# ICLDisco/parsec

Hardware: NVIDIA H100
Metric: tasks/s (higher is better)
Workload: dtype i32

## Files before the change

### parsec_b200/mca/b200/device_b200.h

```cpp
#ifndef PARSEC_DEVICE_B200_H
#define PARSEC_DEVICE_B200_H

#include "parsec/mca/device/device_gpu.h"

BEGIN_C_DECLS

extern parsec_device_base_component_t parsec_device_b200_component;


int parsec_b200_task_body(parsec_device_gpu_module_t *gpu_device, parsec_gpu_task_t *gpu_task,
                          parsec_gpu_exec_stream_t *gpu_stream,
                          int body, int nb_args, const int *flow_index, const int32_t *iparam, float fparam);

uint64_t parsec_b200_task_result(const parsec_gpu_task_t *gpu_task);

int parsec_b200_is_b200_device(const parsec_device_module_t *device);

typedef struct parsec_b200_stats_s {
    uint64_t tasks_engine;
    uint64_t tasks_lane;
    uint64_t kernel_launches;
    uint64_t released_on_device;
    uint64_t bytes_h2d_kernel, bytes_d2d_kernel, bytes_d2h_kernel;
    uint64_t bytes_h2d_dma, bytes_d2h_dma;
    uint64_t evictions, w2r_copies;
    uint64_t registration_hits;
    uint64_t first_entry_ns, first_task_ns, last_done_ns;
    uint64_t peer_pulls;
    uint64_t peer_detours;
    uint64_t check_mismatches;
    uint64_t manager_entries;
    uint64_t lane_batched;
    uint64_t forwarded;
    uint64_t max_concurrent_callers;
} parsec_b200_stats_t;
int parsec_b200_get_stats(const parsec_device_module_t *device, parsec_b200_stats_t *stats);

END_C_DECLS
#endif
```

### parsec_b200/mca/b200/device_b200_component.c

```c
#include "parsec/parsec_config.h"
#include "parsec/parsec_internal.h"
#include "parsec/utils/mca_param.h"
#include "parsec/utils/debug.h"
#include "parsec/constants.h"
#include "parsec/mca/device/device.h"
#include "parsec/mca/device/device_gpu.h"
#include "parsec/mca/device/b200/device_b200.h"
#include "parsec/mca/device/b200/device_b200_internal.h"

#include <stdlib.h>

int parsec_device_b200_enabled = 0;
int parsec_device_b200_enabled_index = -1;
int parsec_b200_dry_run = 0;
int parsec_b200_memory_block_size = 512 * 1024;
int parsec_b200_memory_percentage = 95;
int parsec_b200_memory_number_of_blocks = -1;
int parsec_b200_cmd_slots = 65536;
int parsec_b200_idle_us = 2000;
int parsec_b200_max_workers = 0;
char *parsec_b200_trace = NULL;
int parsec_b200_nvtx = 0;
int parsec_b200_parallel_completion = 1;
int parsec_b200_stage_window = 32 * 1024 * 1024;
int parsec_b200_registration_cache = 1;
static int b200_mask = -1;

#if !defined(PARSEC_HAVE_MPI)
int parsec_mpi_allow_gpu_memory_communications = 0;
#endif

static int device_b200_component_open(void);
static int device_b200_component_close(void);
static int device_b200_component_query(mca_base_module_2_0_0_t **module, int *priority);
static int device_b200_component_register(void);

parsec_device_base_component_t parsec_device_b200_component = {
    {
        PARSEC_DEVICE_BASE_VERSION_2_0_0,
        "b200",
        "+persistent_kernel+device_release+tma",
        PARSEC_VERSION_MAJOR,
        PARSEC_VERSION_MINOR,
        device_b200_component_open,
        device_b200_component_close,
        device_b200_component_query,
        device_b200_component_register,
        "",
// ... 19 lines not shown
    (void)parsec_mca_param_reg_int_name("device_b200", "mask", "Bit mask of the CUDA devices the component may use",
                                        false, false, -1, &b200_mask);
    (void)parsec_mca_param_reg_int_name("device_b200", "dry_run",
                                        "Host-logic test mode: build modules without touching CUDA; tasks retire in dependency order "
                                        "without running their bodies (the value is the number of pretend devices)",
                                        false, false, 0, &parsec_b200_dry_run);
    (void)parsec_mca_param_reg_int_name("device_b200", "memory_block_size", "Unit of the device heap in bytes",
                                        false, false, 512 * 1024, &parsec_b200_memory_block_size);
    (void)parsec_mca_param_reg_int_name("device_b200", "memory_use", "Percentage of the free GPU memory given to the device heap",
                                        false, false, 95, &parsec_b200_memory_percentage);
    (void)parsec_mca_param_reg_int_name("device_b200", "memory_number_of_blocks",
                                        "Exact number of heap blocks instead of a percentage (-1: use device_b200_memory_use)",
                                        false, false, -1, &parsec_b200_memory_number_of_blocks);
    (void)parsec_mca_param_reg_int_name("device_b200", "cmd_slots", "Capacity of the host->device command ring (tasks in flight)",
                                        false, false, 65536, &parsec_b200_cmd_slots);
    (void)parsec_mca_param_reg_int_name("device_b200", "idle_us", "The persistent kernel parks after this many idle microseconds",
                                        false, false, 2000, &parsec_b200_idle_us);
    (void)parsec_mca_param_reg_int_name("device_b200", "parallel_completion",
                                        "Let the worker pool run __parsec_complete_execution of finished GPU tasks instead of the manager thread",
                                        false, false, 1, &parsec_b200_parallel_completion);
    (void)parsec_mca_param_reg_int_name("device_b200", "stage_window",
                                        "Bytes of stage-in (host or peer to device) allowed in flight before further cold tasks wait",
                                        false, false, 32 * 1024 * 1024, &parsec_b200_stage_window);
    (void)parsec_mca_param_reg_int_name("device_b200", "registration_cache",
                                        "Keep host ranges pinned after memory_unregister and revive them at the next registration of the same range",
                                        false, false, 1, &parsec_b200_registration_cache);
    (void)parsec_mca_param_reg_int_name("device_b200", "max_workers", "Debug: limit the worker CTAs of the persistent kernel (0: all)",
                                        false, false, 0, &parsec_b200_max_workers);
    (void)parsec_mca_param_reg_string_name("device_b200", "trace",
                                           "Write one Chrome-trace JSON file <value>.<device index>.json per device at finalize: every task with the "
                                           "device-clock time a worker CTA started and finished it and the SM it ran on (empty: off)",
                                           false, false, "", &parsec_b200_trace);
    (void)parsec_mca_param_reg_int_name("device_b200", "nvtx",
                                        "Wrap the host side of the device in NVTX ranges (domain \"parsec_b200\": start pass, retire pass, "
                                        "epilog batch) and mark every manager election; what profiling_nvtx.c does for the profiling keys "
                                        "of the reference's stream engine",
                                        false, false, 0, &parsec_b200_nvtx);
    return (0 == parsec_device_b200_enabled && 0 == parsec_b200_dry_run) ? MCA_ERROR : MCA_SUCCESS;
}

static int device_b200_component_open(void)
{
    int ndev = 0;
    if( 0 == parsec_device_b200_enabled && 0 == parsec_b200_dry_run ) return MCA_ERROR;
    if( parsec_b200_dry_run > 0 ) {
        ndev = parsec_b200_dry_run;
// ... 52 lines not shown
```

### parsec_b200/mca/b200/device_b200_internal.h

```cpp
#ifndef PARSEC_DEVICE_B200_INTERNAL_H
#define PARSEC_DEVICE_B200_INTERNAL_H

#include "parsec/mca/device/device_gpu.h"
#include "parsec/mca/device/cuda/device_cuda.h"
#include "parsec/mca/device/b200/device_b200.h"

BEGIN_C_DECLS

extern int parsec_device_b200_enabled, parsec_device_b200_enabled_index, parsec_b200_dry_run;
extern int parsec_b200_memory_block_size, parsec_b200_memory_percentage, parsec_b200_memory_number_of_blocks;
extern int parsec_b200_parallel_completion, parsec_b200_stage_window, parsec_b200_registration_cache;
extern char *parsec_b200_trace;
extern int parsec_b200_nvtx;
extern int parsec_b200_cmd_slots, parsec_b200_idle_us, parsec_b200_max_workers;

int  parsec_b200_device_count(void);
int  parsec_b200_module_init(int dev_id, parsec_device_module_t **module);
int  parsec_b200_module_fini(parsec_device_module_t *device);

END_C_DECLS
#endif
```

### parsec_b200/mca/b200/device_b200_module.c

```c
#include "parsec/parsec_config.h"
#include "parsec/parsec_internal.h"
#include "parsec/sys/atomic.h"
#include "parsec/utils/mca_param.h"
#include "parsec/utils/debug.h"
#include "parsec/utils/zone_malloc.h"
#include "parsec/constants.h"
#include "parsec/data_internal.h"
#include "parsec/scheduling.h"
#include "parsec/execution_stream.h"
#include "parsec/mca/device/device.h"
#include "parsec/mca/device/device_gpu.h"
#include "parsec/mca/device/b200/device_b200.h"
#include "parsec/mca/device/b200/device_b200_internal.h"

#include "pb2_engine.h"
#include "pb2_stream.h"

#include <cuda_runtime_api.h>
#include <stddef.h>
#include <stdlib.h>
#include <string.h>
#include <stdio.h>
#include <limits.h>
#include <time.h>
// ... 24 lines not shown

typedef struct b200_lock_s {
    volatile uint32_t next;    char pad0[60];
    volatile uint32_t serving; char pad1[60];
} b200_lock_t;
static inline void b200_lock(b200_lock_t *l)
{
    const uint32_t t = __atomic_fetch_add(&l->next, 1, __ATOMIC_RELAXED);
    while( __atomic_load_n(&l->serving, __ATOMIC_ACQUIRE) != t ) _mm_pause();
}
static inline void b200_unlock(b200_lock_t *l)
{
    __atomic_store_n(&l->serving, l->serving + 1, __ATOMIC_RELEASE);
}

enum {
    BT_NEW = 0,
    BT_STAGED,
    BT_DMA_IN,
    BT_INFLIGHT,
    BT_LANE,
    BT_DMA_OUT
};

typedef struct b200_task_s {
    parsec_list_item_t   item;
    parsec_gpu_task_t   *gpu_task;
    int32_t              state;
    int32_t              ticket;
    int32_t              body;
    int32_t              prepared;
    int32_t              cmd_built;
    int32_t              recorded;
    int32_t              has_complete_stage;
    uint32_t             dma_out_mask;
    uint64_t             result;
    uint64_t             cold_bytes;
    struct parsec_device_b200_module_s *dev;
    int32_t              is_kernel;
    int32_t              defer_tiles;
    int32_t              ntdesc;
    pb2_task_t           cmd __attribute__((aligned(64)));
    parsec_task_t        proxy __attribute__((aligned(64)));
    int32_t              nb_args;
    int32_t              arg_flow[PB2_MAX_FLOWS];
    int32_t              iparam[3];
    float                fparam;
    uint32_t             peer_src_mask;
    parsec_data_copy_t  *peer_src[MAX_PARAM_COUNT];
    int32_t              custom_stage;
    cudaEvent_t          ev;
    int32_t              ev_dev;
    struct b200_task_s  *next_free;
    struct b200_task_s  *next_done;
    struct { int32_t tile; pb2_tile_t desc; } tdesc[MAX_PARAM_COUNT];
} b200_task_t;

typedef struct b200_host_range_s { char *base; size_t len; char *alias; int lazy; } b200_host_range_t;

typedef struct b200_trace_ev_s {
    char     name[24];
    int32_t  locals[2];
    int32_t  body, smid;
    uint64_t t_start_ns, t_end_ns, cold_bytes;
} b200_trace_ev_t;
#define B200_LINE __attribute__((aligned(64)))
typedef struct parsec_device_b200_module_s {
    parsec_device_cuda_module_t super;
    pb2_engine_t        *engine;
    pb2_stream_t        *stream;
    int                  dry_run;
    char                *slab_base;
    uint8_t             *tile_described;
    b200_task_t * volatile *inbox_ring;
    cudaStream_t         dma_stream;
    parsec_cuda_exec_stream_t *lane;
    uint64_t             first_entry_ns, first_task_ns, last_done_ns;
    volatile int64_t     inbox_tail B200_LINE;
    volatile int32_t     owed B200_LINE;
    volatile int32_t     callers_inside B200_LINE;
    volatile int32_t     max_callers_inside;
    volatile int64_t     epilogs_done B200_LINE;
    b200_lock_t          lru_lock B200_LINE;
    b200_lock_t          alloc_lock B200_LINE;
    volatile int32_t     handed_back B200_LINE;
    volatile int32_t     starter_active B200_LINE;
    volatile int32_t     fatal;
    volatile int32_t     memory_pressure;
    struct b200_task_s * volatile lane_done;
    volatile int32_t     retry_stalled B200_LINE;
    volatile int64_t     cold_inflight B200_LINE;
    volatile int64_t     inbox_head B200_LINE;
    parsec_list_t        stalled B200_LINE;
    parsec_list_t        settled;
    parsec_list_t        cold_q;
    int32_t              nb_cold;
    parsec_list_t        waiting_event;
    int32_t              nb_settled;
    int32_t              nb_stalled;
    int32_t              again_window;
    int32_t              lane_pending;
    uint64_t             n_engine, n_lane, n_settled_by_caller;
    uint64_t             tsc_start[4];
    uint64_t             tsc_s[3];
    parsec_list_t        waiting_out B200_LINE;
    parsec_task_t       *completion_ring;
    b200_task_t         *batch_head;
    int32_t              batch_len;
    int32_t              completed_now;
    int32_t              blocked_spins;
    int32_t              complete_inline;
    int64_t              epilogs_started;
    uint64_t             tsc[8];
    struct b200_trace_ev_s *trace_ev;
    size_t               trace_n, trace_cap;
    pb2_retire_t         retbuf[256];
    parsec_b200_stats_t  st B200_LINE;
} parsec_device_b200_module_t;

static b200_host_range_t *b200_ranges = NULL;
// ... 58 lines not shown
{
    b200_task_t *bt = b200_tl_free;
    if( NULL != bt ) { b200_tl_free = bt->next_free; b200_tl_nfree--; }
    else {
        if( 0 != posix_memalign((void**)&bt, 64, sizeof(b200_task_t)) ) abort();
        memset(bt, 0, sizeof(b200_task_t));
        PARSEC_OBJ_CONSTRUCT(&bt->item, parsec_list_item_t);
        PARSEC_OBJ_CONSTRUCT(&bt->proxy, parsec_task_t);
        bt->proxy.task_class = &b200_completion_tc;
        bt->proxy.priority = INT32_MAX;
        bt->proxy.status = PARSEC_TASK_STATUS_HOOK;
        bt->proxy.chore_mask = 1;
        bt->proxy.selected_chore = 0;
        bt->proxy.selected_device = parsec_mca_device_get(0);
        bt->proxy.load = 0;
        bt->proxy.repo_entry = NULL;
        bt->ev_dev = -1;
    }
    PARSEC_LIST_ITEM_SINGLETON(&bt->item);
    bt->dev = dev;
    bt->gpu_task = gpu_task; bt->state = BT_NEW; bt->ticket = -1; bt->body = -1; bt->nb_args = 0;
    bt->peer_src_mask = 0; bt->dma_out_mask = 0; bt->result = 0; bt->custom_stage = 0; bt->cold_bytes = 0;
    bt->recorded = 0; bt->has_complete_stage = 0; bt->prepared = 0; bt->cmd_built = 0; bt->defer_tiles = 0; bt->ntdesc = 0;
    bt->is_kernel = (NULL == gpu_task) || (PARSEC_GPU_TASK_TYPE_KERNEL == gpu_task->task_type);
    if( NULL != gpu_task ) gpu_task->last_data_check_epoch = (uint64_t)(uintptr_t)bt;
    return bt;
}

static void b200_bt_free(b200_task_t *bt)
{
    bt->gpu_task = NULL;
    if( b200_tl_nfree < B200_TL_CACHE ) { bt->next_free = b200_tl_free; b200_tl_free = bt; b200_tl_nfree++; return; }
    if( bt->ev_dev >= 0 ) (void)cudaEventDestroy(bt->ev);
    free(bt);
}

static inline void b200_cuda_here(parsec_device_b200_module_t *dev)
{
    if( !dev->dry_run ) B200_CUDA(cudaSetDevice(dev->super.cuda_index), "cudaSetDevice", {});
}

static cudaEvent_t b200_bt_event(parsec_device_b200_module_t *dev, b200_task_t *bt)
{
    if( bt->ev_dev != (int32_t)dev->super.cuda_index ) {
        if( bt->ev_dev >= 0 ) (void)cudaEventDestroy(bt->ev);
        bt->ev_dev = -1;
// ... 341 lines not shown
        int transfer_from = parsec_data_start_transfer_ownership_to_copy(original, my, type);
        if( -1 != transfer_from && out->version == src->version && PARSEC_DATA_STATUS_COMPLETE_TRANSFER == out->data_transfer_status ) transfer_from = -1;
        if( NULL == src->device_private ) transfer_from = -1;
        if( (NULL == this_task->data[i].source_repo_entry) && (NULL == original->dc) && (0 == in->version) ) transfer_from = -1;
        if( PARSEC_DATA_STATUS_UNDER_TRANSFER == out->data_transfer_status ) transfer_from = -1;
        mod->required_data_in += original->span;

        pb2_tile_t tile;
        memset(&tile, 0, sizeof tile);
        tile.dev_ptr = out->device_private;
        tile.bytes = (uint32_t)span;
        tile.state = PB2_TILE_VALID;
        tile.src_kind = parsec_mca_device_is_gpu(src->device_index) ? PB2_SRC_PEER : PB2_SRC_HOST;
        char *home = NULL;
        if( NULL != original->device_copies[0] && NULL != original->device_copies[0]->device_private )
            home = b200_device_visible(original->device_copies[0]->device_private, span);
        tile.src_ptr = home;

        if( -1 == transfer_from ) {
            if( src_acquired ) { (void)parsec_atomic_fetch_dec_int32(&src->readers); src_acquired = 0; }
            if( PARSEC_DATA_STATUS_UNDER_TRANSFER != out->data_transfer_status ) {
                out->data_transfer_status = PARSEC_DATA_STATUS_COMPLETE_TRANSFER;
                parsec_data_end_transfer_ownership_to_copy(original, my, type);
            }
            if( PARSEC_FLOW_ACCESS_WRITE & type ) out->version = src->version + 1;
        } else {
            char *visible = (PB2_SRC_PEER == tile.src_kind) ? (char*)src->device_private
                                                            : b200_device_visible(src->device_private, span);
            mod->data_in_from_device[src->device_index] += span;
            mod->nb_data_faults += span;
            bt->cold_bytes += span;
            if( PB2_SRC_PEER == tile.src_kind ) { if( src_detour ) dev->st.peer_detours++; else dev->st.peer_pulls++; }
            if( NULL != visible && !src_detour && !for_lane && !dev->dry_run ) {
                tile.state = PB2_TILE_INVALID;
                tile.src_ptr = visible;
                out->data_transfer_status = PARSEC_DATA_STATUS_UNDER_TRANSFER;
                if( PB2_SRC_PEER == tile.src_kind ) dev->st.bytes_d2d_kernel += span; else dev->st.bytes_h2d_kernel += span;
            } else if( 2 == mode ) {
                out->data_transfer_status = PARSEC_DATA_STATUS_UNDER_TRANSFER;
                used_dma = 1;
            } else if( !dev->dry_run ) {
                b200_cuda_here(dev);
                B200_CUDA(cudaMemcpyAsync(out->device_private, src->device_private, span,
                                          PB2_SRC_PEER == tile.src_kind ? cudaMemcpyDeviceToDevice : cudaMemcpyHostToDevice,
                                          for_lane ? dev->lane->cuda_stream : dev->dma_stream),
                          "stage-in cudaMemcpyAsync", { parsec_atomic_unlock(&original->lock); return PARSEC_HOOK_RETURN_ERROR; });
                out->data_transfer_status = PARSEC_DATA_STATUS_UNDER_TRANSFER;
                dev->st.bytes_h2d_dma += span;
                used_dma = 1;
            } else {
                out->data_transfer_status = PARSEC_DATA_STATUS_UNDER_TRANSFER;
            }
            out->version = (PARSEC_FLOW_ACCESS_WRITE & type) ? src->version + 1 : src->version;
            gpu_task->flow_info[i].source = src;
            if( src_acquired ) { bt->peer_src_mask |= (1u << i); bt->peer_src[i] = src; }
            if( PB2_SRC_PEER == tile.src_kind && PB2_TILE_INVALID == tile.state && NULL != home && (gpu_task->pushout & (1 << i)) ) {
            }
        }
        tile.version = (PARSEC_FLOW_ACCESS_WRITE & type) ? out->version - 1 : out->version;
        if( !for_lane ) {
            const int32_t tid = b200_tile_of(dev, out);
            if( -1 != transfer_from || !dev->tile_described[tid] ) {
                if( 0 != b200_emit_tile(dev, bt, tid, &tile) ) { parsec_atomic_unlock(&original->lock); return PARSEC_HOOK_RETURN_ERROR; }
                dev->tile_described[tid] = 1;
            }
        }
        parsec_atomic_unlock(&original->lock);
    }
    return used_dma;
}

int parsec_b200_task_body(parsec_device_gpu_module_t *gpu_device, parsec_gpu_task_t *gpu_task,
                          parsec_gpu_exec_stream_t *gpu_stream,
                          int body, int nb_args, const int *flow_index, const int32_t *iparam, float fparam)
{
    if( NULL == gpu_device || NULL == gpu_task || nb_args < 0 || nb_args > PB2_MAX_FLOWS || body < 0 || body >= PB2_BODY_MAX )
        return PARSEC_HOOK_RETURN_ERROR;
    for( int a = 0; a < nb_args; a++ )
        if( flow_index[a] < 0 || (uint32_t)flow_index[a] >= gpu_task->nb_flows ) return PARSEC_HOOK_RETURN_ERROR;
    if( parsec_b200_is_b200_device(&gpu_device->super) ) {
        b200_task_t *bt = b200_tl_recording;
        if( NULL == bt || bt->gpu_task != gpu_task ) return PARSEC_HOOK_RETURN_ERROR;
        bt->body = body; bt->nb_args = nb_args;
        for( int a = 0; a < nb_args; a++ ) bt->arg_flow[a] = flow_index[a];
        bt->iparam[0] = iparam ? iparam[0] : 0; bt->iparam[1] = iparam ? iparam[1] : 0; bt->iparam[2] = iparam ? iparam[2] : 0;
        bt->fparam = fparam;
        return PARSEC_HOOK_RETURN_DONE;
    }
    {
        void *ptrs[PB2_MAX_FLOWS] = {NULL, NULL, NULL, NULL};
        uint64_t bytes[PB2_MAX_FLOWS] = {0, 0, 0, 0};
// ... 183 lines not shown
            NULL != gpu_task->ec->data[f].data_out ) bt->dma_out_mask |= (1u << f);
    }
    t->iparam[0] = bt->iparam[0]; t->iparam[1] = bt->iparam[1]; t->iparam[2] = bt->iparam[2]; t->fparam = bt->fparam;
    t->locals[0] = gpu_task->ec->locals[0].value; t->locals[1] = gpu_task->ec->locals[1].value;
    bt->cmd_built = 1;
}

static int b200_push_engine(parsec_device_b200_module_t *dev, b200_task_t *bt)
{
    if( !bt->cmd_built ) b200_build_cmd(dev, bt);
    const int32_t state_before = bt->state;
    bt->state = BT_INFLIGHT;
    int rc = pb2_stream_submit(dev->stream, &bt->cmd, (uint64_t)(uintptr_t)bt, &bt->ticket);
    if( PB2_SUCCESS != rc ) {
        bt->state = state_before;
        if( PB2_ERR_OUT_OF_RESOURCE == rc ) return PARSEC_HOOK_RETURN_AGAIN;
        parsec_warning("device_b200: submit failed: %s", pb2_stream_last_error(dev->stream));
        return PARSEC_HOOK_RETURN_ERROR;
    }
    dev->n_engine++;
    return PARSEC_HOOK_RETURN_DONE;
}

static int b200_prepare_resident(parsec_device_b200_module_t *dev, b200_task_t *bt)
{
    parsec_gpu_task_t *gpu_task = bt->gpu_task;
    parsec_task_t *this_task = gpu_task->ec;
    const uint8_t my = dev->super.super.super.device_index;
    if( NULL == dev->tile_described ) return 0;
    for( uint32_t i = 0; i < gpu_task->nb_flows; i++ ) {
        const parsec_flow_t *flow = gpu_task->flow_info[i].flow;
        if( PARSEC_FLOW_ACCESS_NONE == (PARSEC_FLOW_ACCESS_MASK & flow->flow_flags) ) continue;
        const parsec_data_copy_t *in = this_task->data[i].data_in;
        if( NULL == in ) continue;
        if( in->device_index != my || NULL == in->device_private || NULL == in->original ) return 0;
        if( !dev->tile_described[b200_tile_of(dev, in)] ) return 0;
    }
    for( uint32_t i = 0; i < gpu_task->nb_flows; i++ ) {
        const parsec_flow_t *flow = gpu_task->flow_info[i].flow;
        const uint8_t type = (uint8_t)(flow->flow_flags & PARSEC_FLOW_ACCESS_MASK);
        if( PARSEC_FLOW_ACCESS_NONE == type ) { gpu_task->flow_info[i].flow_span = 0; continue; }
        parsec_data_copy_t *in = this_task->data[i].data_in;
        if( NULL == in ) continue;
        this_task->data[i].data_out = in;
        gpu_task->flow_info[i].source = NULL;
        if( PARSEC_FLOW_ACCESS_WRITE & type ) {
// ... 96 lines not shown

static int b200_start_task(parsec_device_b200_module_t *dev, parsec_execution_stream_t *es, b200_task_t *bt)
{
    parsec_gpu_task_t *gpu_task = bt->gpu_task;
    int rc;
    (void)es;
    dev->again_window = 0;
    if( bt->prepared ) { bt->state = BT_STAGED; return b200_push_engine(dev, bt); }
    if( dev->cold_inflight >= (int64_t)parsec_b200_stage_window && b200_needs_memory(dev, gpu_task) ) { dev->again_window = 1; return PARSEC_HOOK_RETURN_AGAIN; }
    uint64_t c0 = B200_TSC(), c1;
    if( PARSEC_HOOK_RETURN_DONE != (rc = b200_reserve(dev, bt)) ) return rc;
    c1 = B200_TSC(); dev->tsc_start[0] += c1 - c0; c0 = c1;

    const int custom_stage = (NULL != gpu_task->stage_in && gpu_task->stage_in != parsec_default_gpu_stage_in) ||
                             (NULL != gpu_task->stage_out && gpu_task->stage_out != parsec_default_gpu_stage_out);
    const parsec_task_class_t *tc = gpu_task->ec->task_class;
    bt->custom_stage = custom_stage;
    int known_engine = bt->recorded || dev->dry_run || (!custom_stage && parsec_b200_submit_is_engine(gpu_task->submit));

    if( known_engine ) {
        rc = b200_stage_in(dev, bt, 0);
        if( rc < 0 ) return rc;
        c1 = B200_TSC(); dev->tsc_start[1] += c1 - c0; c0 = c1;
        if( bt->cold_bytes ) (void)parsec_atomic_fetch_add_int64(&dev->cold_inflight, (int64_t)bt->cold_bytes);
        int src = 0;
        if( !bt->recorded ) {
            b200_tl_recording = bt;
            src = gpu_task->submit(&dev->super.super, gpu_task, &dev->lane->super);
            b200_tl_recording = NULL;
            bt->recorded = 1;
            bt->has_complete_stage = (NULL != gpu_task->complete_stage);
        }
        if( dev->dry_run && bt->body < 0 ) { bt->body = PB2_BODY_NOP; bt->nb_args = 0; }
        if( src < 0 || bt->body < 0 ) {
            parsec_warning("device_b200: body of task class %s stopped naming an engine body", tc ? tc->name : "?");
            return PARSEC_HOOK_RETURN_ERROR;
        }
        if( rc > 0 ) {
            B200_CUDA(cudaEventRecord(b200_bt_event(dev, bt), dev->dma_stream), "cudaEventRecord", {});
            bt->state = BT_DMA_IN;
            parsec_list_nolock_push_back(&dev->waiting_event, &bt->item);
            return PARSEC_HOOK_RETURN_DONE;
        }
        bt->state = BT_STAGED;
        c1 = B200_TSC(); dev->tsc_start[2] += c1 - c0; c0 = c1;
        rc = b200_push_engine(dev, bt);
        dev->tsc_start[3] += B200_TSC() - c0;
        return rc;
    }

    b200_cuda_here(dev);
    const int user_in = (NULL != gpu_task->stage_in && gpu_task->stage_in != parsec_default_gpu_stage_in);
    rc = b200_stage_in(dev, bt, user_in ? 2 : 1);
    if( rc < 0 ) return rc;
    if( bt->cold_bytes ) (void)parsec_atomic_fetch_add_int64(&dev->cold_inflight, (int64_t)bt->cold_bytes);
    if( user_in ) {
        uint32_t mask = 0;
        for( uint32_t i = 0; i < gpu_task->nb_flows; i++ )
            if( NULL != gpu_task->ec->data[i].data_out && PARSEC_DATA_STATUS_UNDER_TRANSFER == gpu_task->ec->data[i].data_out->data_transfer_status ) mask |= (1u << i);
        if( mask && PARSEC_SUCCESS != gpu_task->stage_in(gpu_task, mask, &dev->lane->super) ) return PARSEC_HOOK_RETURN_ERROR;
// ... 69 lines not shown
        gpu_task->ec = (parsec_task_t*)calloc(1, sizeof(parsec_task_t));
        PARSEC_OBJ_CONSTRUCT(gpu_task->ec, parsec_task_t);
        gpu_task->ec->task_class = &b200_prefetch_tc;
        gpu_task->ec->selected_device = module;
        gpu_task->nb_flows = 1;
        gpu_task->flow_info[0].flow = &b200_prefetch_flow;
        gpu_task->flow_info[0].flow_span = data->span;
        gpu_task->stage_in = parsec_default_gpu_stage_in;
        gpu_task->stage_out = parsec_default_gpu_stage_out;
        gpu_task->submit = b200_prefetch_submit;
        gpu_task->release_device_task = b200_release_pseudo_task;
        PARSEC_DATA_COPY_RETAIN(src);
        gpu_task->ec->data[0].data_in = src;
        (void)b200_kernel_scheduler(module, NULL, gpu_task);
        return PARSEC_SUCCESS;
    }
    default:
        return PARSEC_ERR_NOT_FOUND;
    }
}

static void b200_finish(parsec_device_b200_module_t *dev, parsec_execution_stream_t *es, b200_task_t *bt)
{
    if( bt->cold_bytes ) { (void)parsec_atomic_fetch_add_int64(&dev->cold_inflight, -(int64_t)bt->cold_bytes); bt->cold_bytes = 0; }
    if( !dev->retry_stalled ) dev->retry_stalled = 1;
    if( bt->is_kernel ) { b200_complete(dev, es, bt); return; }
    parsec_gpu_task_t *gpu_task = bt->gpu_task;
    parsec_data_copy_t *out = gpu_task->ec->data[0].data_out;
    if( NULL != out ) {
        parsec_atomic_lock(&out->original->lock);
        if( PARSEC_DATA_STATUS_UNDER_TRANSFER == out->data_transfer_status ) {
            out->data_transfer_status = PARSEC_DATA_STATUS_COMPLETE_TRANSFER;
            parsec_data_end_transfer_ownership_to_copy(out->original, dev->super.super.super.device_index, PARSEC_FLOW_ACCESS_READ);
        }
        if( bt->peer_src_mask & 1u ) (void)parsec_atomic_fetch_dec_int32(&bt->peer_src[0]->readers);
        if( 1 == out->readers ) b200_lru_touch(dev, out);
        (void)parsec_atomic_fetch_dec_int32(&out->readers);
        parsec_atomic_unlock(&out->original->lock);
    }
    b200_bt_free(bt);
    gpu_task->last_data_check_epoch = 0;
    gpu_task->release_device_task(gpu_task);
    dev->completed_now++;
}

static parsec_device_b200_module_t *b200_forward_peer(parsec_device_b200_module_t *dev, const parsec_gpu_task_t *gpu_task)
{
// ... 87 lines not shown
        dev->retry_stalled = 0;
        while( dev->nb_settled > 0 ) {
            if( started >= 512 ) { cut = 1; break; }
            b200_task_t *bt = (b200_task_t*)PARSEC_LIST_ITERATOR_FIRST(&dev->settled);
            parsec_list_item_t *la = PARSEC_LIST_ITERATOR_NEXT(&bt->item);
            if( la != PARSEC_LIST_ITERATOR_END(&dev->settled) ) { la = PARSEC_LIST_ITERATOR_NEXT(la);
                if( la != PARSEC_LIST_ITERATOR_END(&dev->settled) ) { B200_PF(la); B200_PF((const char*)la + offsetof(b200_task_t, cmd)); } }
            parsec_list_nolock_remove(&dev->settled, &bt->item);
            PARSEC_LIST_ITEM_SINGLETON(&bt->item);
            if( BT_NEW == bt->state ) bt->state = BT_STAGED;
            const int rc = b200_push_engine(dev, bt);
            if( PARSEC_HOOK_RETURN_AGAIN == rc ) { parsec_list_nolock_push_front(&dev->settled, &bt->item); ring_full = 1; break; }
            if( PARSEC_HOOK_RETURN_DONE != rc ) return -1;
            dev->nb_settled--;
            started++;
        }
        while( !ring_full && !cut && dev->nb_cold > 0 ) {
            if( started >= 512 ) { cut = 1; break; }
            b200_task_t *bt = (b200_task_t*)PARSEC_LIST_ITERATOR_FIRST(&dev->cold_q);
            if( bt->cold_bytes && dev->cold_inflight >= (int64_t)parsec_b200_stage_window ) break;
            parsec_list_nolock_remove(&dev->cold_q, &bt->item);
            PARSEC_LIST_ITEM_SINGLETON(&bt->item);
            if( BT_NEW == bt->state ) bt->state = BT_STAGED;
            const uint64_t cold = bt->cold_bytes;
            const int rc = b200_push_engine(dev, bt);
            if( PARSEC_HOOK_RETURN_AGAIN == rc ) { parsec_list_nolock_push_front(&dev->cold_q, &bt->item); ring_full = 1; break; }
            if( PARSEC_HOOK_RETURN_DONE != rc ) return -1;
            if( cold ) (void)parsec_atomic_fetch_add_int64(&dev->cold_inflight, (int64_t)cold);
            dev->nb_cold--;
            started++;
        }
        parsec_list_item_t *it = PARSEC_LIST_ITERATOR_FIRST(&dev->stalled), *next;
        int mem_blocked = 0;
        for( ; !ring_full && !cut && it != PARSEC_LIST_ITERATOR_END(&dev->stalled); it = next ) {
            b200_task_t *bt = (b200_task_t*)it;
            next = PARSEC_LIST_ITERATOR_NEXT(it);
            int rc;
            if( started >= 512 ) { cut = 1; break; }
            if( next != PARSEC_LIST_ITERATOR_END(&dev->stalled) ) {
                parsec_list_item_t *la = next;
                b200_pf4((b200_task_t*)la); la = PARSEC_LIST_ITERATOR_NEXT(la);
                if( la != PARSEC_LIST_ITERATOR_END(&dev->stalled) ) { b200_pf3((b200_task_t*)la); la = PARSEC_LIST_ITERATOR_NEXT(la);
                if( la != PARSEC_LIST_ITERATOR_END(&dev->stalled) ) { b200_pf2((b200_task_t*)la); la = PARSEC_LIST_ITERATOR_NEXT(la);
                if( la != PARSEC_LIST_ITERATOR_END(&dev->stalled) ) { b200_pf1((b200_task_t*)la); } } }
            }
            if( mem_blocked && BT_NEW == bt->state && b200_needs_memory(dev, bt->gpu_task) ) {
// ... 4 lines not shown
            PARSEC_LIST_ITEM_SINGLETON(it);
            if( BT_NEW == bt->state ) {
                b200_lock(&dev->alloc_lock);
                const int n = b200_drain_inbox(dev);
                rc = (n < 0) ? PARSEC_HOOK_RETURN_ERROR : b200_start_task(dev, es, bt);
                b200_unlock(&dev->alloc_lock);
                if( n > 0 ) moved += n;
            } else rc = b200_push_engine(dev, bt);
            if( PARSEC_HOOK_RETURN_AGAIN == rc ) {
                if( next == PARSEC_LIST_ITERATOR_END(&dev->stalled) ) parsec_list_nolock_push_back(&dev->stalled, it);
                else parsec_list_nolock_add_before(&dev->stalled, next, it);
                if( BT_NEW != bt->state ) break;
                if( dev->again_window ) break;
                if( b200_hand_back(dev, es, bt) ) { moved++; continue; }
                mem_blocked = 1;
                continue;
            }
            if( PARSEC_HOOK_RETURN_DONE != rc ) return -1;
            dev->nb_stalled--;
            started++;
        }
        if( cut ) dev->retry_stalled = 1;
    }
    if( dev->lane_pending > 0 ) { const int n = b200_fire_lane(dev); if( n < 0 ) return -1; moved += n; }
    if( started && PB2_SUCCESS != pb2_stream_kick(dev->stream) ) return -1;
    t1 = B200_TSC(); dev->tsc_s[1] += t1 - t0; t0 = t1;
    if( !parsec_list_nolock_is_empty(&dev->waiting_event) ) {
        parsec_list_item_t *it = PARSEC_LIST_ITERATOR_FIRST(&dev->waiting_event), *next;
        for( ; it != PARSEC_LIST_ITERATOR_END(&dev->waiting_event); it = next ) {
            b200_task_t *bt = (b200_task_t*)it;
            next = PARSEC_LIST_ITERATOR_NEXT(it);
            cudaError_t q = cudaEventQuery(bt->ev);
            if( cudaErrorNotReady == q ) { (void)cudaGetLastError(); continue; }
            if( cudaSuccess != q ) { parsec_warning("device_b200: event failed: %s", cudaGetErrorString(q)); return -1; }
            parsec_list_nolock_remove(&dev->waiting_event, it);
            PARSEC_LIST_ITEM_SINGLETON(it);
            if( BT_DMA_IN == bt->state ) {
                parsec_gpu_task_t *gt = bt->gpu_task;
                for( uint32_t i = 0; i < gt->nb_flows; i++ ) {
                    parsec_data_copy_t *out = gt->ec->data[i].data_out;
                    if( NULL == out || NULL == gt->ec->data[i].data_in || PARSEC_DATA_STATUS_UNDER_TRANSFER != out->data_transfer_status ) continue;
                    parsec_atomic_lock(&out->original->lock);
                    out->data_transfer_status = PARSEC_DATA_STATUS_COMPLETE_TRANSFER;
                    parsec_data_end_transfer_ownership_to_copy(out->original, dev->super.super.super.device_index,
                                                               (uint8_t)(gt->flow_info[i].flow->flow_flags & PARSEC_FLOW_ACCESS_MASK));
                    parsec_atomic_unlock(&out->original->lock);
                }
                bt->state = BT_STAGED;
                int rc = b200_push_engine(dev, bt);
                if( PARSEC_HOOK_RETURN_AGAIN == rc ) { parsec_list_nolock_push_front(&dev->stalled, &bt->item); dev->nb_stalled++; dev->retry_stalled = 1; }
                else if( PARSEC_HOOK_RETURN_DONE != rc ) return -1;
                else if( PB2_SUCCESS != pb2_stream_kick(dev->stream) ) return -1;
            } else {
                b200_task_t *old;
                do { old = dev->lane_done; bt->next_done = old; } while( !parsec_atomic_cas_ptr(&dev->lane_done, old, bt) );
            }
            moved++;
        }
    }
    t1 = B200_TSC(); dev->tsc_s[2] += t1 - t0; t0 = t1;
    return moved + started;
}

static void b200_trace_task(parsec_device_b200_module_t *dev, const b200_task_t *bt, const pb2_retire_t *r)
{
    if( dev->trace_n == dev->trace_cap ) {
        dev->trace_cap = dev->trace_cap ? 2 * dev->trace_cap : 65536;
        dev->trace_ev = (b200_trace_ev_t*)realloc(dev->trace_ev, dev->trace_cap * sizeof(b200_trace_ev_t));
    }
    b200_trace_ev_t *e = &dev->trace_ev[dev->trace_n++];
    const parsec_task_t *t = bt->gpu_task->ec;
    memset(e, 0, sizeof *e);
    snprintf(e->name, sizeof e->name, "%s", (NULL != t && NULL != t->task_class && NULL != t->task_class->name) ? t->task_class->name : "?");
    if( NULL != t ) { e->locals[0] = t->locals[0].value; e->locals[1] = t->locals[1].value; }
    e->body = bt->body; e->smid = (int32_t)r->smid; e->t_start_ns = r->t_start_ns; e->t_end_ns = r->t_end_ns; e->cold_bytes = bt->cold_bytes;
}

static void b200_trace_write(parsec_device_b200_module_t *dev)
{
    if( NULL == dev->trace_ev || 0 == dev->trace_n || NULL == parsec_b200_trace || '\0' == parsec_b200_trace[0] ) return;
    char path[1024];
// ... 54 lines not shown
            bt->result = dev->retbuf[i].result;
            if( NULL != dev->trace_ev || (NULL != parsec_b200_trace && '\0' != parsec_b200_trace[0]) ) b200_trace_task(dev, bt, &dev->retbuf[i]);
            if( (PB2_BODY_CHECK_I32 == bt->body || PB2_BODY_CHECK_F32 == bt->body) && (bt->result >> 32) ) dev->st.check_mismatches += bt->result >> 32;
            bt->ticket = -1;
            if( PB2_SUCCESS != dev->retbuf[i].status ) { parsec_warning("device_b200: task ran an unknown engine body"); return -1; }
            if( bt->dma_out_mask && b200_dma_pushout(dev, bt) > 0 ) {
                bt->state = BT_DMA_OUT;
                parsec_list_nolock_push_back(&dev->waiting_out, &bt->item);
            } else b200_finish(dev, es, bt);
        }
        if( n > 0 ) b200_nvtx_pop();
        t1 = B200_TSC(); dev->tsc[4] += t1 - t0; t0 = t1;
        if( n < (int)(sizeof(dev->retbuf) / sizeof(dev->retbuf[0])) ) break;
    }
    dev->complete_inline = 0;
    b200_close_batch(dev);
    return 0;
}

static inline int b200_start_work(const parsec_device_b200_module_t *dev)
{
    return dev->inbox_tail != dev->inbox_head ||
           ((dev->nb_stalled > 0 || dev->nb_settled > 0 || dev->nb_cold > 0) && dev->retry_stalled) ||
           !parsec_list_nolock_is_empty((parsec_list_t*)&dev->waiting_event);
}

static int b200_try_start(parsec_device_b200_module_t *dev, parsec_execution_stream_t *es, int sticky)
{
    for(;;) {
        if( dev->starter_active || !parsec_atomic_cas_int32(&dev->starter_active, 0, 1) ) return 0;
        int rc;
        do { b200_nvtx_push("b200 start pass"); rc = b200_start_pass(dev, es); b200_nvtx_pop(); } while( rc > 0 && sticky );
        if( rc < 0 ) dev->fatal = 1;
        parsec_atomic_wmb();
        dev->starter_active = 0;
        parsec_mfence();
        if( rc < 0 ) return -1;
        if( dev->inbox_tail == dev->inbox_head ) return 0;
    }
}


static parsec_hook_return_t
b200_kernel_scheduler(parsec_device_module_t *module, parsec_execution_stream_t *es, void *_gpu_task)
{
    parsec_device_b200_module_t *dev = (parsec_device_b200_module_t*)module;
    parsec_gpu_task_t *gpu_task = (parsec_gpu_task_t*)_gpu_task;
// ... 311 lines not shown
    gpu->memory_allocate  = b200_memory_allocate;
    gpu->memory_free      = b200_memory_free;
    gpu->find_incarnation = b200_find_incarnation;
    device->gflops_fp16 = 989000; device->gflops_tf32 = 495000; device->gflops_fp32 = 67000; device->gflops_fp64 = 34000;
    device->gflops_guess = 0;
    device->device_load = 0;

    PARSEC_OBJ_CONSTRUCT(&gpu->gpu_mem_lru, parsec_list_t);
    PARSEC_OBJ_CONSTRUCT(&gpu->gpu_mem_owned_lru, parsec_list_t);
    PARSEC_OBJ_CONSTRUCT(&gpu->pending, parsec_fifo_t);
    PARSEC_OBJ_CONSTRUCT(&dev->stalled, parsec_list_t);
    PARSEC_OBJ_CONSTRUCT(&dev->settled, parsec_list_t);
    PARSEC_OBJ_CONSTRUCT(&dev->waiting_out, parsec_list_t);
    PARSEC_OBJ_CONSTRUCT(&dev->cold_q, parsec_list_t);
    PARSEC_OBJ_CONSTRUCT(&dev->waiting_event, parsec_list_t);
    memset(&dev->lru_lock, 0, sizeof dev->lru_lock);
    dev->inbox_ring = (b200_task_t * volatile *)calloc(B200_INBOX_SLOTS, sizeof(b200_task_t*));

    int nblocks = parsec_b200_memory_number_of_blocks;
    if( dev->dry_run && -1 == nblocks ) nblocks = 4096;
    if( PARSEC_SUCCESS != parsec_device_memory_reserve(gpu, parsec_b200_memory_percentage, nblocks, (size_t)parsec_b200_memory_block_size) ) goto failed;

    dev->tile_described = (uint8_t*)calloc((size_t)gpu->mem_nb_blocks + 1, 1);
    pb2_stream_params_t sp;
    memset(&sp, 0, sizeof sp);
    sp.cmd_slots = parsec_b200_cmd_slots;
    sp.max_tiles = (int32_t)gpu->mem_nb_blocks;
    sp.idle_us = parsec_b200_idle_us;
    sp.dry_run = dev->dry_run;
    sp.max_workers = parsec_b200_max_workers;
    sp.trace = (NULL != parsec_b200_trace && '\0' != parsec_b200_trace[0]);
    if( parsec_b200_nvtx && NULL == b200_nvtx_domain ) b200_nvtx_domain = nvtxDomainCreateA("parsec_b200");
    if( PB2_SUCCESS != pb2_stream_create(dev->engine, &sp, &dev->stream) ) goto failed;
    *module = device;
    return PARSEC_SUCCESS;
failed:
    parsec_warning("device_b200: initialisation of device %d failed", dev_id);
    if( NULL != dev->engine ) pb2_engine_destroy(dev->engine);
    free(device->name); free(dev);
    return PARSEC_ERROR;
}

int parsec_b200_module_fini(parsec_device_module_t *device)
{
    parsec_device_b200_module_t *dev = (parsec_device_b200_module_t*)device;
    parsec_device_gpu_module_t *gpu = &dev->super.super;
    if( NULL != dev->stream ) { (void)pb2_stream_quiesce(dev->stream); }
    b200_profile_print(dev);
    b200_trace_write(dev);
    free(dev->trace_ev); dev->trace_ev = NULL; dev->trace_n = dev->trace_cap = 0;
    while( dev->epilogs_done < dev->epilogs_started ) { parsec_atomic_rmb(); }
    while( b200_write_back_some(dev, 64) > 0 ) { }
    parsec_device_memory_release(gpu);
    b200_registration_cache_drop(dev);
    if( NULL != dev->stream ) { pb2_stream_destroy(dev->stream); dev->stream = NULL; }
    free((void*)dev->inbox_ring); dev->inbox_ring = NULL;
    PARSEC_OBJ_DESTRUCT(&gpu->pending);
    PARSEC_OBJ_DESTRUCT(&dev->lane->super.infos);
    free(dev->lane->super.name);
    PARSEC_OBJ_RELEASE(dev->lane->super.fifo_pending);
    if( !dev->dry_run ) {
        (void)cudaStreamDestroy(dev->lane->cuda_stream);
        (void)cudaStreamDestroy(dev->dma_stream);
    }
    free(dev->tile_described);
    free(dev->lane); free(gpu->exec_stream);
    if( NULL != dev->engine ) { pb2_engine_destroy(dev->engine); dev->engine = NULL; }
    free(device->name); device->name = NULL;
    return PARSEC_SUCCESS;
}
```

Measured before the change: 98.30 million.

## Stage registered host tiles through copy engine in coalesced batches

Host-sourced input tiles of engine tasks are no longer pulled by the persistent kernel. They are copied by the copy engine, grouped into batches that are flushed at a byte threshold or when the start pass drains. Each batch sorts its copies, merges strided runs into 1D/2D memcpys, issues the rest through cudaMemcpyBatchAsync, and records one event per batch. This is meant to free worker CTAs from host reads and cut per-copy API overhead, at the cost of extra host bookkeeping, per-tile sequence tracking and added stage-in latency while a batch fills.

```diff
diff --git a/parsec_b200/mca/b200/device_b200.h b/parsec_b200/mca/b200/device_b200.h
--- a/parsec_b200/mca/b200/device_b200.h
+++ b/parsec_b200/mca/b200/device_b200.h
@@ -33,6 +33,7 @@
     uint64_t lane_batched;
     uint64_t forwarded;
     uint64_t max_concurrent_callers;
+    uint64_t dma_batches;
 } parsec_b200_stats_t;
 int parsec_b200_get_stats(const parsec_device_module_t *device, parsec_b200_stats_t *stats);
 
diff --git a/parsec_b200/mca/b200/device_b200_component.c b/parsec_b200/mca/b200/device_b200_component.c
--- a/parsec_b200/mca/b200/device_b200_component.c
+++ b/parsec_b200/mca/b200/device_b200_component.c
@@ -24,6 +24,7 @@
 int parsec_b200_parallel_completion = 1;
 int parsec_b200_stage_window = 32 * 1024 * 1024;
 int parsec_b200_registration_cache = 1;
+int parsec_b200_dma_stage_in_batch = 4 * 1024 * 1024;
 static int b200_mask = -1;
 
 #if !defined(PARSEC_HAVE_MPI)
@@ -89,6 +90,10 @@
     (void)parsec_mca_param_reg_int_name("device_b200", "stage_window",
                                         "Bytes of stage-in (host or peer to device) allowed in flight before further cold tasks wait",
                                         false, false, 32 * 1024 * 1024, &parsec_b200_stage_window);
+    (void)parsec_mca_param_reg_int_name("device_b200", "dma_stage_in_batch",
+                                        "Registered host tiles that engine tasks read come in through the copy engine, in batches issued once they "
+                                        "hold this many bytes or when no more tasks wait to be staged (0: the persistent kernel pulls them)",
+                                        false, false, 4 * 1024 * 1024, &parsec_b200_dma_stage_in_batch);
     (void)parsec_mca_param_reg_int_name("device_b200", "registration_cache",
                                         "Keep host ranges pinned after memory_unregister and revive them at the next registration of the same range",
                                         false, false, 1, &parsec_b200_registration_cache);
diff --git a/parsec_b200/mca/b200/device_b200_internal.h b/parsec_b200/mca/b200/device_b200_internal.h
--- a/parsec_b200/mca/b200/device_b200_internal.h
+++ b/parsec_b200/mca/b200/device_b200_internal.h
@@ -9,7 +9,7 @@
 
 extern int parsec_device_b200_enabled, parsec_device_b200_enabled_index, parsec_b200_dry_run;
 extern int parsec_b200_memory_block_size, parsec_b200_memory_percentage, parsec_b200_memory_number_of_blocks;
-extern int parsec_b200_parallel_completion, parsec_b200_stage_window, parsec_b200_registration_cache;
+extern int parsec_b200_parallel_completion, parsec_b200_stage_window, parsec_b200_registration_cache, parsec_b200_dma_stage_in_batch;
 extern char *parsec_b200_trace;
 extern int parsec_b200_nvtx;
 extern int parsec_b200_cmd_slots, parsec_b200_idle_us, parsec_b200_max_workers;
diff --git a/parsec_b200/mca/b200/device_b200_module.c b/parsec_b200/mca/b200/device_b200_module.c
--- a/parsec_b200/mca/b200/device_b200_module.c
+++ b/parsec_b200/mca/b200/device_b200_module.c
@@ -70,6 +70,8 @@
     BT_LANE,
     BT_DMA_OUT
 };
+
+typedef struct b200_ce_copy_s { char *dst; const char *src; size_t bytes; } b200_ce_copy_t;
 
 typedef struct b200_task_s {
     parsec_list_item_t   item;
@@ -102,7 +104,21 @@
     struct b200_task_s  *next_free;
     struct b200_task_s  *next_done;
     struct { int32_t tile; pb2_tile_t desc; } tdesc[MAX_PARAM_COUNT];
+    int32_t              nce;
+    int32_t              cold_landed;
+    int64_t              ce_seq;
+    struct b200_task_s  *next_in_batch;
+    b200_ce_copy_t       ce[MAX_PARAM_COUNT];
 } b200_task_t;
+
+typedef struct b200_ce_batch_s {
+    struct b200_ce_batch_s *next;
+    b200_task_t         *head, *tail;
+    int64_t              seq;
+    uint64_t             bytes;
+    cudaEvent_t          ev;
+    int32_t              has_ev;
+} b200_ce_batch_t;
 
 typedef struct b200_host_range_s { char *base; size_t len; char *alias; int lazy; } b200_host_range_t;
 
@@ -120,6 +136,8 @@
     int                  dry_run;
     char                *slab_base;
     uint8_t             *tile_described;
+    int64_t             *tile_ce_seq;
+    int64_t              ce_decided;
     b200_task_t * volatile *inbox_ring;
     cudaStream_t         dma_stream;
     parsec_cuda_exec_stream_t *lane;
@@ -144,6 +162,13 @@
     parsec_list_t        cold_q;
     int32_t              nb_cold;
     parsec_list_t        waiting_event;
+    b200_ce_batch_t     *ce_open;
+    b200_ce_batch_t     *ce_first, *ce_last;
+    b200_ce_batch_t     *ce_free;
+    int64_t              ce_landed;
+    b200_ce_copy_t      *ce_scratch;
+    void               **ce_dsts, **ce_srcs;
+    size_t              *ce_sizes, ce_cap;
     int32_t              nb_settled;
     int32_t              nb_stalled;
     int32_t              again_window;
@@ -248,6 +273,7 @@
     bt->gpu_task = gpu_task; bt->state = BT_NEW; bt->ticket = -1; bt->body = -1; bt->nb_args = 0;
     bt->peer_src_mask = 0; bt->dma_out_mask = 0; bt->result = 0; bt->custom_stage = 0; bt->cold_bytes = 0;
     bt->recorded = 0; bt->has_complete_stage = 0; bt->prepared = 0; bt->cmd_built = 0; bt->defer_tiles = 0; bt->ntdesc = 0;
+    bt->nce = 0; bt->cold_landed = 0; bt->ce_seq = 0;
     bt->is_kernel = (NULL == gpu_task) || (PARSEC_GPU_TASK_TYPE_KERNEL == gpu_task->task_type);
     if( NULL != gpu_task ) gpu_task->last_data_check_epoch = (uint64_t)(uintptr_t)bt;
     return bt;
@@ -635,6 +661,8 @@
             if( PARSEC_DATA_STATUS_UNDER_TRANSFER != out->data_transfer_status ) {
                 out->data_transfer_status = PARSEC_DATA_STATUS_COMPLETE_TRANSFER;
                 parsec_data_end_transfer_ownership_to_copy(original, my, type);
+            } else if( !for_lane && dev->tile_ce_seq[b200_tile_of(dev, out)] > bt->ce_seq ) {
+                bt->ce_seq = dev->tile_ce_seq[b200_tile_of(dev, out)];
             }
             if( PARSEC_FLOW_ACCESS_WRITE & type ) out->version = src->version + 1;
         } else {
@@ -644,7 +672,13 @@
             mod->nb_data_faults += span;
             bt->cold_bytes += span;
             if( PB2_SRC_PEER == tile.src_kind ) { if( src_detour ) dev->st.peer_detours++; else dev->st.peer_pulls++; }
-            if( NULL != visible && !src_detour && !for_lane && !dev->dry_run ) {
+            if( NULL != visible && PB2_SRC_HOST == tile.src_kind && !for_lane && parsec_b200_dma_stage_in_batch > 0 ) {
+                bt->ce[bt->nce].dst = (char*)out->device_private; bt->ce[bt->nce].src = (const char*)src->device_private;
+                bt->ce[bt->nce].bytes = span; bt->nce++;
+                dev->tile_ce_seq[b200_tile_of(dev, out)] = dev->ce_decided + 1;
+                out->data_transfer_status = PARSEC_DATA_STATUS_UNDER_TRANSFER;
+                dev->st.bytes_h2d_dma += span;
+            } else if( NULL != visible && !src_detour && !for_lane && !dev->dry_run ) {
                 tile.state = PB2_TILE_INVALID;
                 tile.src_ptr = visible;
                 out->data_transfer_status = PARSEC_DATA_STATUS_UNDER_TRANSFER;
@@ -680,6 +714,15 @@
         }
         parsec_atomic_unlock(&original->lock);
     }
+    if( bt->nce ) {
+        bt->ce_seq = ++dev->ce_decided;
+        if( used_dma ) {
+            for( int c = 0; c < bt->nce; c++ )
+                B200_CUDA(cudaMemcpyAsync(bt->ce[c].dst, bt->ce[c].src, bt->ce[c].bytes, cudaMemcpyHostToDevice, dev->dma_stream),
+                          "stage-in cudaMemcpyAsync", { return PARSEC_HOOK_RETURN_ERROR; });
+            bt->nce = 0;
+        }
+    }
     return used_dma;
 }
 
@@ -909,6 +952,124 @@
     return PARSEC_HOOK_RETURN_DONE;
 }
 
+static inline int b200_ce_waits(const parsec_device_b200_module_t *dev, const b200_task_t *bt)
+{
+    return bt->nce > 0 || bt->ce_seq > dev->ce_landed;
+}
+
+static void b200_ce_add(parsec_device_b200_module_t *dev, b200_task_t *bt)
+{
+    b200_ce_batch_t *b = dev->ce_open;
+    if( NULL == b ) {
+        if( NULL != (b = dev->ce_free) ) dev->ce_free = b->next;
+        else if( NULL == (b = (b200_ce_batch_t*)calloc(1, sizeof *b)) ) abort();
+        b->next = NULL; b->head = b->tail = NULL; b->seq = 0; b->bytes = 0;
+        dev->ce_open = b;
+    }
+    bt->next_in_batch = NULL;
+    if( NULL == b->tail ) b->head = bt; else b->tail->next_in_batch = bt;
+    b->tail = bt;
+    if( bt->ce_seq > b->seq ) b->seq = bt->ce_seq;
+    b->bytes += bt->cold_bytes;
+}
+
+static int b200_ce_cmp(const void *a, const void *b)
+{
+    const char *x = ((const b200_ce_copy_t*)a)->dst, *y = ((const b200_ce_copy_t*)b)->dst;
+    return (x > y) - (x < y);
+}
+
+static int b200_ce_flush(parsec_device_b200_module_t *dev)
+{
+    b200_ce_batch_t *b = dev->ce_open;
+    if( NULL == b ) return 0;
+    dev->ce_open = NULL;
+    if( !dev->dry_run ) {
+        size_t n = 0;
+        for( b200_task_t *bt = b->head; NULL != bt; bt = bt->next_in_batch ) n += (size_t)bt->nce;
+        if( n > dev->ce_cap ) {
+            dev->ce_cap = 2 * n;
+            dev->ce_scratch = (b200_ce_copy_t*)realloc(dev->ce_scratch, dev->ce_cap * sizeof(b200_ce_copy_t));
+            dev->ce_dsts = (void**)realloc(dev->ce_dsts, dev->ce_cap * sizeof(void*));
+            dev->ce_srcs = (void**)realloc(dev->ce_srcs, dev->ce_cap * sizeof(void*));
+            dev->ce_sizes = (size_t*)realloc(dev->ce_sizes, dev->ce_cap * sizeof(size_t));
+            if( NULL == dev->ce_scratch || NULL == dev->ce_dsts || NULL == dev->ce_srcs || NULL == dev->ce_sizes ) abort();
+        }
+        b200_ce_copy_t *c = dev->ce_scratch;
+        n = 0;
+        for( b200_task_t *bt = b->head; NULL != bt; bt = bt->next_in_batch )
+            for( int k = 0; k < bt->nce; k++ ) c[n++] = bt->ce[k];
+        qsort(c, n, sizeof *c, b200_ce_cmp);
+        b200_cuda_here(dev);
+        size_t nsingle = 0;
+        for( size_t i = 0, j; i < n; i = j ) {
+            const ptrdiff_t w = (ptrdiff_t)c[i].bytes;
+            ptrdiff_t dp = 0, hp = 0;
+            j = i + 1;
+            if( j < n && c[j].bytes == c[i].bytes ) { dp = c[j].dst - c[i].dst; hp = c[j].src - c[i].src; }
+            if( dp >= w && hp >= w && dp <= INT_MAX && hp <= INT_MAX )
+                while( j < n && c[j].bytes == c[i].bytes && c[j].dst - c[j - 1].dst == dp && c[j].src - c[j - 1].src == hp ) j++;
+            if( j - i >= 2 && NULL == b200_device_visible(c[i].src, (size_t)hp * (j - i - 1) + (size_t)w) ) j = i + 1;
+            if( j - i < 2 ) { dev->ce_dsts[nsingle] = c[i].dst; dev->ce_srcs[nsingle] = (void*)c[i].src; dev->ce_sizes[nsingle++] = c[i].bytes; continue; }
+            if( dp == w && hp == w )
+                B200_CUDA(cudaMemcpyAsync(c[i].dst, c[i].src, (size_t)w * (j - i), cudaMemcpyHostToDevice, dev->dma_stream),
+                          "stage-in batch cudaMemcpyAsync", { return -1; });
+            else
+                B200_CUDA(cudaMemcpy2DAsync(c[i].dst, (size_t)dp, c[i].src, (size_t)hp, (size_t)w, j - i, cudaMemcpyHostToDevice, dev->dma_stream),
+                          "stage-in batch cudaMemcpy2DAsync", { return -1; });
+        }
+        if( 1 == nsingle ) {
+            B200_CUDA(cudaMemcpyAsync(dev->ce_dsts[0], dev->ce_srcs[0], dev->ce_sizes[0], cudaMemcpyHostToDevice, dev->dma_stream),
+                      "stage-in batch cudaMemcpyAsync", { return -1; });
+        } else if( nsingle > 1 ) {
+            struct cudaMemcpyAttributes attr;
+            size_t attr_idx = 0, fail_idx = 0;
+            memset(&attr, 0, sizeof attr);
+            attr.srcAccessOrder = cudaMemcpySrcAccessOrderStream;
+            B200_CUDA(cudaMemcpyBatchAsync(dev->ce_dsts, dev->ce_srcs, dev->ce_sizes, nsingle, &attr, &attr_idx, 1, &fail_idx, dev->dma_stream),
+                      "stage-in cudaMemcpyBatchAsync", { return -1; });
+        }
+        if( !b->has_ev ) {
+            B200_CUDA(cudaEventCreateWithFlags(&b->ev, cudaEventDisableTiming), "cudaEventCreate", { return -1; });
+            b->has_ev = 1;
+        }
+        B200_CUDA(cudaEventRecord(b->ev, dev->dma_stream), "cudaEventRecord", { return -1; });
+    }
+    if( NULL == dev->ce_last ) dev->ce_first = b; else dev->ce_last->next = b;
+    dev->ce_last = b;
+    dev->st.dma_batches++;
+    return 0;
+}
+
+static int b200_ce_land(parsec_device_b200_module_t *dev)
+{
+    int moved = 0;
+    b200_ce_batch_t *b;
+    while( NULL != (b = dev->ce_first) ) {
+        if( !dev->dry_run ) {
+            const cudaError_t q = cudaEventQuery(b->ev);
+            if( cudaErrorNotReady == q ) { (void)cudaGetLastError(); break; }
+            if( cudaSuccess != q ) { parsec_warning("device_b200: stage-in batch failed: %s", cudaGetErrorString(q)); return -1; }
+        }
+        dev->ce_first = b->next;
+        if( NULL == dev->ce_first ) dev->ce_last = NULL;
+        if( b->seq > dev->ce_landed ) dev->ce_landed = b->seq;
+        if( b->bytes ) (void)parsec_atomic_fetch_add_int64(&dev->cold_inflight, -(int64_t)b->bytes);
+        for( b200_task_t *bt = b->head, *next; NULL != bt; bt = next ) {
+            next = bt->next_in_batch;
+            bt->nce = 0; bt->cold_landed = 1;
+            bt->state = BT_STAGED;
+            const int rc = b200_push_engine(dev, bt);
+            if( PARSEC_HOOK_RETURN_AGAIN == rc ) { parsec_list_nolock_push_back(&dev->stalled, &bt->item); dev->nb_stalled++; dev->retry_stalled = 1; }
+            else if( PARSEC_HOOK_RETURN_DONE != rc ) return -1;
+            moved++;
+        }
+        b->next = dev->ce_free; dev->ce_free = b;
+    }
+    if( moved && PB2_SUCCESS != pb2_stream_kick(dev->stream) ) return -1;
+    return moved;
+}
+
 static int b200_prepare_resident(parsec_device_b200_module_t *dev, b200_task_t *bt)
 {
     parsec_gpu_task_t *gpu_task = bt->gpu_task;
@@ -1051,7 +1212,6 @@
         rc = b200_stage_in(dev, bt, 0);
         if( rc < 0 ) return rc;
         c1 = B200_TSC(); dev->tsc_start[1] += c1 - c0; c0 = c1;
-        if( bt->cold_bytes ) (void)parsec_atomic_fetch_add_int64(&dev->cold_inflight, (int64_t)bt->cold_bytes);
         int src = 0;
         if( !bt->recorded ) {
             b200_tl_recording = bt;
@@ -1065,6 +1225,14 @@
             parsec_warning("device_b200: body of task class %s stopped naming an engine body", tc ? tc->name : "?");
             return PARSEC_HOOK_RETURN_ERROR;
         }
+        if( 0 == rc && b200_ce_waits(dev, bt) ) {
+            bt->state = BT_STAGED;
+            parsec_list_nolock_push_back(&dev->cold_q, &bt->item);
+            dev->nb_cold++;
+            dev->retry_stalled = 1;
+            return PARSEC_HOOK_RETURN_DONE;
+        }
+        if( bt->cold_bytes ) (void)parsec_atomic_fetch_add_int64(&dev->cold_inflight, (int64_t)bt->cold_bytes);
         if( rc > 0 ) {
             B200_CUDA(cudaEventRecord(b200_bt_event(dev, bt), dev->dma_stream), "cudaEventRecord", {});
             bt->state = BT_DMA_IN;
@@ -1180,7 +1348,7 @@
 
 static void b200_finish(parsec_device_b200_module_t *dev, parsec_execution_stream_t *es, b200_task_t *bt)
 {
-    if( bt->cold_bytes ) { (void)parsec_atomic_fetch_add_int64(&dev->cold_inflight, -(int64_t)bt->cold_bytes); bt->cold_bytes = 0; }
+    if( bt->cold_bytes && !bt->cold_landed ) { (void)parsec_atomic_fetch_add_int64(&dev->cold_inflight, -(int64_t)bt->cold_bytes); bt->cold_bytes = 0; }
     if( !dev->retry_stalled ) dev->retry_stalled = 1;
     if( bt->is_kernel ) { b200_complete(dev, es, bt); return; }
     parsec_gpu_task_t *gpu_task = bt->gpu_task;
@@ -1314,6 +1482,13 @@
             parsec_list_nolock_remove(&dev->cold_q, &bt->item);
             PARSEC_LIST_ITEM_SINGLETON(&bt->item);
             if( BT_NEW == bt->state ) bt->state = BT_STAGED;
+            if( b200_ce_waits(dev, bt) ) {
+                if( bt->cold_bytes ) (void)parsec_atomic_fetch_add_int64(&dev->cold_inflight, (int64_t)bt->cold_bytes);
+                b200_ce_add(dev, bt);
+                dev->nb_cold--;
+                if( dev->ce_open->bytes >= (uint64_t)parsec_b200_dma_stage_in_batch && b200_ce_flush(dev) < 0 ) return -1;
+                continue;
+            }
             const uint64_t cold = bt->cold_bytes;
             const int rc = b200_push_engine(dev, bt);
             if( PARSEC_HOOK_RETURN_AGAIN == rc ) { parsec_list_nolock_push_front(&dev->cold_q, &bt->item); ring_full = 1; break; }
@@ -1364,9 +1539,15 @@
         }
         if( cut ) dev->retry_stalled = 1;
     }
+    if( b200_ce_flush(dev) < 0 ) return -1;
     if( dev->lane_pending > 0 ) { const int n = b200_fire_lane(dev); if( n < 0 ) return -1; moved += n; }
     if( started && PB2_SUCCESS != pb2_stream_kick(dev->stream) ) return -1;
     t1 = B200_TSC(); dev->tsc_s[1] += t1 - t0; t0 = t1;
+    if( NULL != dev->ce_first ) {
+        const int n = b200_ce_land(dev);
+        if( n < 0 ) return -1;
+        moved += n;
+    }
     if( !parsec_list_nolock_is_empty(&dev->waiting_event) ) {
         parsec_list_item_t *it = PARSEC_LIST_ITERATOR_FIRST(&dev->waiting_event), *next;
         for( ; it != PARSEC_LIST_ITERATOR_END(&dev->waiting_event); it = next ) {
@@ -1389,6 +1570,7 @@
                     parsec_atomic_unlock(&out->original->lock);
                 }
                 bt->state = BT_STAGED;
+                if( b200_ce_waits(dev, bt) ) { b200_ce_add(dev, bt); moved++; continue; }
                 int rc = b200_push_engine(dev, bt);
                 if( PARSEC_HOOK_RETURN_AGAIN == rc ) { parsec_list_nolock_push_front(&dev->stalled, &bt->item); dev->nb_stalled++; dev->retry_stalled = 1; }
                 else if( PARSEC_HOOK_RETURN_DONE != rc ) return -1;
@@ -1399,6 +1581,7 @@
             }
             moved++;
         }
+        if( b200_ce_flush(dev) < 0 ) return -1;
     }
     t1 = B200_TSC(); dev->tsc_s[2] += t1 - t0; t0 = t1;
     return moved + started;
@@ -1499,7 +1682,7 @@
 {
     return dev->inbox_tail != dev->inbox_head ||
            ((dev->nb_stalled > 0 || dev->nb_settled > 0 || dev->nb_cold > 0) && dev->retry_stalled) ||
-           !parsec_list_nolock_is_empty((parsec_list_t*)&dev->waiting_event);
+           !parsec_list_nolock_is_empty((parsec_list_t*)&dev->waiting_event) || NULL != dev->ce_first;
 }
 
 static int b200_try_start(parsec_device_b200_module_t *dev, parsec_execution_stream_t *es, int sticky)
@@ -1857,6 +2040,7 @@
     if( PARSEC_SUCCESS != parsec_device_memory_reserve(gpu, parsec_b200_memory_percentage, nblocks, (size_t)parsec_b200_memory_block_size) ) goto failed;
 
     dev->tile_described = (uint8_t*)calloc((size_t)gpu->mem_nb_blocks + 1, 1);
+    dev->tile_ce_seq = (int64_t*)calloc((size_t)gpu->mem_nb_blocks + 1, sizeof(int64_t));
     pb2_stream_params_t sp;
     memset(&sp, 0, sizeof sp);
     sp.cmd_slots = parsec_b200_cmd_slots;
@@ -1899,6 +2083,13 @@
         (void)cudaStreamDestroy(dev->dma_stream);
     }
     free(dev->tile_described);
+    free(dev->tile_ce_seq);
+    for( b200_ce_batch_t *b = dev->ce_free, *next; NULL != b; b = next ) {
+        next = b->next;
+        if( b->has_ev && !dev->dry_run ) (void)cudaEventDestroy(b->ev);
+        free(b);
+    }
+    free(dev->ce_scratch); free(dev->ce_dsts); free(dev->ce_srcs); free(dev->ce_sizes);
     free(dev->lane); free(gpu->exec_stream);
     if( NULL != dev->engine ) { pb2_engine_destroy(dev->engine); dev->engine = NULL; }
     free(device->name); device->name = NULL;
```

After: 99.58 million, median of 6. About the same (+1.3%).
